# CTPLab/Tera-MIND

Hardware: AMD Instinct MI355X
Metric: denoising steps/sec on 64x64x(2 stains x 2 z) patches (interior patch-steps/s) (higher is better)
Workload: dtype f32; 1 GPU; configs[1]: b=32 images x 1 interior 64x64 patch (P=1, 128 padded + 32 collage patches/step), rna_slc=4, rna_num=229, stain=all, DDPM T=50 schedule, f32, mode A (pad+patchify -> UNet -> DDPM update); parallelism=dp1 (independent patch batches)

## Files before the change

### include/teramind_hip.h

```cpp
#ifndef TERAMIND_HIP_H
#define TERAMIND_HIP_H

#include <stddef.h>
#include <stdint.h>

#ifdef __cplusplus
extern "C" {
#endif

#define TM_ABI_VERSION 1

enum {
  TM_OK = 0,
  TM_ERR_ARG = -1,
  TM_ERR_STATE = -2,
  TM_ERR_KEY = -3,
  TM_ERR_HIP = -4,
  TM_ERR_WORKSPACE = -5
};

enum { TM_DTYPE_F32 = 0, TM_DTYPE_BF16 = 1, TM_DTYPE_F16 = 2 };
enum { TM_SAMPLE_DDPM = 0, TM_SAMPLE_DDIM = 1 };

typedef struct tm_config {
// ... 138 lines not shown
  double total_ms;
  double nominal_flops;
  double executed_flops;
  double alg_bytes;
} tm_prof_stats;
int tm_profile_enable(tm_model* m, int on);
int tm_profile_collect(tm_model* m, tm_prof_stats* out);


int tm_op_to_cb8(const void* x_ncdhw, void* y_cb8, int N, int C, int Z, int H, int W, void* stream);
int tm_op_from_cb8(const void* x_cb8, void* y_ncdhw, int N, int C, int Z, int H, int W, void* stream);

int tm_op_conv_mfma(const void* x_cb8, const void* w_host, const void* bias_host, void* y_cb8,
                    int N, int Cin, int Cout, int Z, int S, int ksize, int zmode, int up2,
                    int tile_variant, void* stream);
int tm_op_conv_mfma_res(const void* x_cb8, const void* w_host, const void* bias_host, void* y_cb8, const void* res_cb8,
                        int res_half, int N, int Cin, int Cout, int Z, int S, int ksize, int zmode, int up2,
                        int tile_variant, void* stream);

int tm_op_conv_zpair_fused_f32(const void* x_cb8, const void* w_host, const void* bias_host, const void* norm_w_host,
                               const void* scale_host, const void* shift_host, const void* res_cb8, void* a2_out,
                               void* h1_out, void* a2_sep_out, int N, int Cin, int Cout, int Z, int S, int per_image,
                               int tile_variant, void* stream);

int tm_op_conv_ups_pair_f32(const void* x_cb8, const void* w_host, const void* bias_host, void* y_cb8, int N, int Cin,
                            int Cout, int Z, int S, int tile_variant, void* stream);

int tm_op_conv_xpair_f32(const void* x_cb8, const void* w_host, const void* bias_host, void* y_cb8, const void* res_cb8,
                         int res_half, int N, int Cin, int Cout, int Z, int S, int tile_variant, void* stream);
int tm_op_conv_pad1_time_f32(const void* x_cb8, const void* w_host, const void* bias_host, void* y_cb8, int N, int Cin,
                             int Cout, int S, int form, int tile_variant, int iters, float* ms_out, void* stream);

int tm_op_conv1_f32(const void* x_cb8, const void* w_host, const void* bias_host, void* y_cb8, const void* res_cb8,
                    const void* gate_cb8, int x_cbtot, int x_cb0, int gate_cbtot, int gate_cb0, int gate_half, int gelu,
                    int tile_variant, int N, int Cin, int Cout, int Z, int S, int* form_out, void* stream);
int tm_conv1_form(long vox, int ntile, int tile_variant);

int tm_conv_frag_addrs(int kernel, int half, int tw, int what, int wave, int p, int ky, int kx, int sub, int* out64);

int tm_op_conv27_bf16(const void* x_cb8, const void* w_host, const void* bias_host, void* y_cb8,
                      int N, int Cin, int Cout, int S, int dtype, int waves, const void* res_h16, void* y_h16,
                      int ups, int res_half, void* stream);
int tm_op_conv27_h16_z(const void* x_cb8, const void* w_host, const void* bias_host, void* y_cb8,
                       int N, int Cin, int Cout, int S, int dtype, int waves, const void* res_h16, void* y_h16,
                       int ups, int res_half, int Z, void* stream);

// ... 135 lines not shown
```

### tera-mind_amd/_lib.py

```python
import ctypes as C
import os

_HERE = os.path.dirname(os.path.abspath(__file__))
LIB_PATH = os.environ.get("TM_LIB_PATH") or os.path.join(_HERE, "csrc", "libteramind_hip.so")

c_void_p, c_int, c_size_t, c_char_p, c_float = C.c_void_p, C.c_int, C.c_size_t, C.c_char_p, C.c_float
c_i64_p = C.POINTER(C.c_int64)


class TmConfig(C.Structure):
    _fields_ = [("patch_size", C.c_int32), ("rna_slc", C.c_int32), ("n_stain", C.c_int32),
                ("rna_num", C.c_int32), ("net_ch", C.c_int32), ("ch_mult", C.c_int32 * 4),
                ("embed_ch", C.c_int32), ("attn_res", C.c_int32), ("num_res_blocks", C.c_int32),
                ("vis_only", C.c_int32), ("dtype", C.c_int32)]


class TmStepCoefs(C.Structure):
    _fields_ = [("sqrt_recip_alphas_cumprod", c_float), ("sqrt_recipm1_alphas_cumprod", c_float),
                ("posterior_mean_coef1", c_float), ("posterior_mean_coef2", c_float),
                ("sigma", c_float), ("sqrt_alpha_bar_prev", c_float),
                ("sqrt_one_minus_alpha_bar_prev", c_float)]


class TmProfStats(C.Structure):
# ... 50 lines not shown
                                        C.c_int64, c_void_p, c_void_p]),
    "tm_blosc_frame_info": (c_int, [c_void_p, c_size_t, c_void_p]),
    "tm_blosc_decompress_dev": (c_int, [c_void_p, c_void_p, c_void_p, c_int, c_void_p, C.c_int64, c_void_p, c_void_p, c_void_p]),
    "tm_blosc_decompress_tiles": (c_int, [c_void_p, c_void_p, c_void_p, c_int, c_void_p, c_int] + [C.c_int64] * 3 + [c_void_p] * 3),
    "tm_u8_shrink2": (c_int, [c_void_p, c_int, c_int, C.c_int64, c_void_p, C.c_int64, c_void_p]),
    "tm_jpeg_encode_tiles": (c_int, [c_void_p, c_int, c_int, C.c_int64] + [c_int] * 3 + [c_void_p, C.c_int64] + [c_void_p] * 4),
    "tm_jpeg_tables": (c_int, [c_int, c_void_p, c_size_t, C.POINTER(c_size_t)]),
    "tm_ssim_planes": (c_int, [c_void_p, c_void_p] + [c_int] * 4 + [C.c_int64] * 4 + [C.POINTER(c_float), c_int, c_float, c_float, c_void_p, c_void_p]),
    "tm_avgpool2_pad": (c_int, [c_void_p] + [c_int] * 4 + [C.c_int64] * 2 + [c_void_p] + [C.c_int64] * 2 + [c_void_p]),
    "tm_profile_enable": (c_int, [c_void_p, c_int]),
    "tm_profile_collect": (c_int, [c_void_p, C.POINTER(TmProfStats)]),
    "tm_op_to_cb8": (c_int, [c_void_p, c_void_p, c_int, c_int, c_int, c_int, c_int, c_void_p]),
    "tm_op_from_cb8": (c_int, [c_void_p, c_void_p, c_int, c_int, c_int, c_int, c_int, c_void_p]),
    "tm_op_conv_mfma": (c_int, [c_void_p, c_void_p, c_void_p, c_void_p] + [c_int] * 9 + [c_void_p]),
    "tm_op_conv_mfma_res": (c_int, [c_void_p, c_void_p, c_void_p, c_void_p, c_void_p] + [c_int] * 10 + [c_void_p]),
    "tm_op_conv1_f32": (c_int, [c_void_p] * 6 + [c_int] * 12 + [C.POINTER(c_int), c_void_p]),
    "tm_conv1_form": (c_int, [C.c_long, c_int, c_int]),
    "tm_conv_frag_addrs": (c_int, [c_int] * 9 + [c_void_p]),
    "tm_op_conv27_bf16": (c_int, [c_void_p, c_void_p, c_void_p, c_void_p] + [c_int] * 6 + [c_void_p] * 2 + [c_int] * 2 + [c_void_p]),
    "tm_op_conv27_fused": (c_int, [c_void_p] * 7 + [c_int] * 7 + [c_void_p]),
    "tm_op_conv27_h16_z": (c_int, [c_void_p, c_void_p, c_void_p, c_void_p] + [c_int] * 6 + [c_void_p] * 2 + [c_int] * 3 + [c_void_p]),
    "tm_op_conv27_fused_z": (c_int, [c_void_p] * 7 + [c_int] * 8 + [c_void_p]),
    "tm_op_conv_zpair_fused_f32": (c_int, [c_void_p] * 10 + [c_int] * 7 + [c_void_p]),
    "tm_op_conv_ups_pair_f32": (c_int, [c_void_p] * 4 + [c_int] * 6 + [c_void_p]),
    "tm_op_conv_xpair_f32": (c_int, [c_void_p] * 5 + [c_int] * 7 + [c_void_p]),
    "tm_op_conv_pad1_time_f32": (c_int, [c_void_p] * 4 + [c_int] * 7 + [C.POINTER(c_float), c_void_p]),
    "tm_op_conv27_time":(c_int, [c_int] * 10 + [c_void_p, c_void_p]),
    "tm_op_conv1_bf16": (c_int, [c_void_p, c_void_p, c_void_p, c_void_p] + [c_int] * 8 + [c_void_p] * 4),
    "tm_op_conv1_h16_gate": (c_int, [c_void_p, c_void_p, c_void_p, c_void_p] + [c_int] * 8 + [c_void_p] * 3 + [c_int] * 3 + [c_void_p]),
    "tm_op_conv1_concat": (c_int, [c_void_p, c_void_p, c_void_p, c_int, c_void_p, c_void_p, c_void_p] + [c_int] * 8 + [c_void_p]),
    "tm_op_prep_h16": (c_int, [c_void_p] * 3 + [c_int] * 7 + [c_void_p, c_int, c_int, c_void_p, c_void_p, C.c_long] +
                       [c_int] * 4 + [c_void_p, c_void_p, c_int, c_void_p, c_void_p]),
    "tm_op_prep_f32": (c_int, [c_void_p] * 3 + [c_int] * 7 + [c_void_p, c_int, c_int, c_void_p, c_void_p, C.c_long] +
                       [c_int] * 4 + [c_void_p, c_void_p, c_int, c_void_p, c_void_p]),
    "tm_op_prep_form": (c_int, [c_void_p] * 3 + [c_int] * 9 + [c_void_p, c_int, c_int, c_int, c_void_p, c_void_p, C.c_long] +
                        [c_int] * 5 + [c_void_p, c_void_p, c_int, c_int, c_void_p, c_void_p]),
    "tm_op_stem": (c_int, [c_void_p] * 4 + [c_int] * 6 + [c_void_p]),
    "tm_op_head": (c_int, [c_void_p] * 4 + [c_int] * 6 + [c_void_p]),
    "tm_op_time_embed": (c_int, [c_void_p] * 7 + [c_int] * 3 + [c_void_p]),
    "tm_op_emb_all": (c_int, [c_void_p] * 4 + [c_int] * 3 + [c_void_p]),
    "tm_op_prep_train": (c_int, [c_void_p] * 5 + [c_float, c_int, c_void_p] + [c_int] * 4 + [c_void_p]),
    "tm_op_prep_bwd": (c_int, [c_void_p] * 6 + [c_float, c_int] + [c_void_p] * 4 + [c_int] * 4 + [c_void_p]),
    "tm_op_prep_train_rng": (c_int, [c_void_p] * 4 + [C.c_uint64, C.c_uint, c_float, c_int, c_void_p] + [c_int] * 4 + [c_void_p]),
    "tm_op_prep_bwd_rng": (c_int, [c_void_p] * 5 + [C.c_uint64, C.c_uint, c_float, c_int] + [c_void_p] * 4 + [c_int] * 4 + [c_void_p]),
    "tm_op_dropout_mask": (c_int, [C.c_uint64, C.c_uint, c_float, c_void_p] + [c_int] * 4 + [c_void_p]),
    "tm_op_conv_dgrad": (c_int, [c_void_p, c_void_p, c_void_p] + [c_int] * 6 + [c_void_p]),
# ... 63 lines not shown
```

### tera-mind_amd/csrc/tm_conv_pack.cpp

```cpp
#include "tm_conv_frag.h"
#include "tm_kernels.h"

#include <stdlib.h>
#include <string.h>

#include <vector>

namespace tmk {

int conv_form_taps(int form) {
  switch (form) {
    case CF_1X1: return 1;
    case CF_INPLANE: return 9;
    case CF_ZSKIP_UPS: case CF_PAIR_UPS: return 12;
    case CF_XPAIR: return 36;
    default: return 27;
  }
}
static bool form_ups(int form) { return form == CF_ZSKIP_UPS || form == CF_PAIR_UPS; }
size_t conv_pack_floats(int form, int Cout, int Cbi) {
  return (size_t)(form_ups(form) ? 4 : 1) * ((Cout + 63) / 64) * Cbi * conv_form_taps(form) * 512;
}
ConvW conv_w(int form, int Cout, int Cbi) {
  ConvW cw;
  cw.form = form; cw.Cout = Cout; cw.Cbi = Cbi; cw.taps = conv_form_taps(form); cw.ntile = (Cout + 63) / 64;
  return cw;
}

static bool switch_on(const char* name) {
  const char* v = getenv(name);
  return !(v && atoi(v) == 0);
}
int conv_pick_form(int ksize, int zmode, int Z, bool deep8, int role, bool* fuse_mid) {
  static const bool zpair_on = switch_on("TM_CONV_ZPAIR"), xpair_on = switch_on("TM_CONV_XPAIR"),
                    xmid_on = switch_on("TM_CONV_XPAIR_MID"), fuse_on = switch_on("TM_CONV_FUSE_MID");
  if (fuse_mid) *fuse_mid = false;
  if (ksize == 1) return CF_1X1;
  if (zmode == ZM_INPLANE) return CF_INPLANE;
  if (zmode == ZM_VALID) return CF_PLANES3;
  const bool pair = Z == 2 && zpair_on;
  if (zmode == ZM_UPS) return ((role & ROLE_OP_PAIR_UPS) || ((role & ROLE_RES) && pair)) ? CF_PAIR_UPS : CF_ZSKIP_UPS;
  if (Z != 2) return (Z == 1 && (role & ROLE_RES)) ? CF_INPLANE : CF_PLANES3;
  if ((role & ROLE_OP_XPAIR) && xpair_on) return CF_XPAIR;
  if (!pair) return CF_ZSKIP;
  const bool fuses = (role & ROLE_C1_64) && fuse_on;
  const bool xp = (role & ROLE_RES) && !(role & ROLE_DEEP) && xpair_on && deep8 && (!fuses || xmid_on);
  if (fuse_mid) *fuse_mid = fuses && !xp;
  return xp ? CF_XPAIR : CF_PAIR;
}

static void seg_counts(const int* seg_c, int nseg, int& Cin, int& Cbi) {
  Cin = Cbi = 0;
  for (int s = 0; s < nseg; ++s) { Cin += seg_c[s]; Cbi += (seg_c[s] + 7) / 8; }
}
static void pack_taps(const float* w, int Cout, const int* seg_c, int nseg, int taps, float* out, bool halves = false) {
  int Cin, Cbi;
  seg_counts(seg_c, nseg, Cin, Cbi);
  memset(out, 0, (size_t)((Cout + 63) / 64) * Cbi * taps * 512 * sizeof(float));
  int ci0 = 0, cb0 = 0;
  for (int s = 0; s < nseg; ++s) {
    for (int c = 0; c < seg_c[s]; ++c) {
      const int ci = ci0 + c;
      const int cb = cb0 + c / 8, c8 = c % 8;
      for (int co = 0; co < Cout; ++co) {
        const int nt = co / 64, col = co % 64;
        const float* src = w + ((size_t)co * Cin + ci) * taps;
        float* dst = out + (((size_t)nt * Cbi + cb) * taps) * 512 + (halves ? conv_w_off(col, c8) : col * 8 + c8);
        for (int t = 0; t < taps; ++t) dst[(size_t)t * 512] = src[t];
      }
    }
// ... 88 lines not shown
```

### tera-mind_amd/csrc/tm_device.h

```cpp
#pragma once
#include "tm_kernels.h"
#include <math.h>
#include <atomic>

namespace tmk {

typedef float f32x4 __attribute__((ext_vector_type(4)));
typedef float f32x16 __attribute__((ext_vector_type(16)));

#define TM_EPS 1e-6f

struct DevOnce {
  std::atomic<unsigned long long> done[2] = {{0ull}, {0ull}};
  static int dev() { int d = -1; return hipGetDevice(&d) == hipSuccess ? d : -1; }
  bool need() const {
    const int d = dev();
    if (d < 0 || d >= 128) return true;
    return !((done[d >> 6].load(std::memory_order_acquire) >> (d & 63)) & 1ull);
  }
  void mark() {
    const int d = dev();
    if (d >= 0 && d < 128) done[d >> 6].fetch_or(1ull << (d & 63), std::memory_order_release);
  }
};
// ... 184 lines not shown
  const float t = h ? t1 : t0;
  if (ooff < 0) return;
  const float rstd = 1.0f / sqrtf(t * a.inv_c + TM_EPS);
  const long mo = (long)(n / a.per_image) * a.mod_stride;
  float* yp = a.y + (long)n * a.y_nstride + ooff + 4 * h;
#pragma unroll
  for (int ct = 0; ct < 2; ++ct)
#pragma unroll
    for (int g = 0; g < 4; ++g) {
      const int c0 = (ct * 4 + g) * 8 + 4 * h;
      const f32x4 wn = *(const f32x4*)(a.norm_w + c0);
      const f32x4 sc = *(const f32x4*)(a.mod_scale + mo + c0), sh = *(const f32x4*)(a.mod_shift + mo + c0);
      f32x4 r;
#pragma unroll
      for (int j = 0; j < 4; ++j) {
        float v = wn[j] * (o[ct][0][4 * g + j] * rstd);
        v = v * (1.0f + sc[j]) + sh[j];
        r[j] = silu_h16(v);
      }
      *(f32x4*)(yp + (long)(ct * 4 + g) * a.y_plane) = r;
    }
}

}
```

### tera-mind_amd/csrc/tm_kernels.h

```cpp
#pragma once
#include <hip/hip_runtime.h>
#include <stdint.h>

#include <vector>

#include "../../include/teramind_hip.h"

namespace tmk {

struct TV {
  float* p = nullptr;
  int N = 0, C = 0, Cb = 0, Z = 0, H = 0, W = 0;
  long nstride = 0;
  long plane() const { return (long)Z * H * W * 8; }
  TV blocks(int cb0, int ncb) const {
    TV v = *this;
    v.p = p + (long)cb0 * plane();
    v.Cb = ncb;
    v.C = ncb * 8;
    return v;
  }
};
inline TV cb8_view(void* p, int N, int C, int Z, int H, int W) {
  TV t;
// ... 37 lines not shown
enum { EPI_NONE = 0, EPI_GELU = 1, EPI_UP2 = 2 };
enum { ZM_PAD1 = 0, ZM_INPLANE = 1, ZM_VALID = 2,
       ZM_UPS = 3 };
struct ConvLaunch {
  TV x;
  ConvW w;
  TV y;
  const TV* res = nullptr;
  const TV* gate = nullptr;
  int flags = 0;
  int tile_variant = 0;
  int gate_half = 0;
  int res_half = 0;
  int zmode = ZM_PAD1;
  int fuse_norm = 0;
  const float *norm_w = nullptr, *mod_scale = nullptr, *mod_shift = nullptr;
  float inv_c = 0.f;
  long mod_stride = 0;
  int per_image = 1;
  TV a2;
};
hipError_t launch_conv_mfma(const ConvLaunch& L, hipStream_t s);
int conv_tile(int form, long ovox, int ntile, int S, int tile_variant);
int conv_frag_addrs(int kernel, int half, int tw, int what, int wv, int p, int ky, int kx, int sub, int* out);
int conv1_form(long vox, int ntile, int tile_variant);

struct TVH {
  uint16_t* p = nullptr;
  int N = 0, C = 0, Cb = 0, Z = 0, H = 0, W = 0;
  long nstride = 0;
  TVH blocks(int cb0, int ncb) const {
    TVH t = *this;
    t.p = p + (long)cb0 * Z * H * W * 8;
    t.Cb = ncb; t.C = ncb * 8;
    return t;
  }
};
struct ConvLaunchH {
  TVH x;
  const uint16_t* w = nullptr;
  const float* bias = nullptr;
  int Cout = 0;
  TV y;
  const TV* res = nullptr;
  const TV* gate = nullptr;
  const TVH* gate_h = nullptr;
// ... 291 lines not shown
```

### tera-mind_amd/csrc/tm_kernels.hip

```cpp
#include "tm_conv_pair.h"

#include <stdlib.h>
#include <string.h>

#include <type_traits>

namespace tmk {

template <int NZI, int WM, int TW, bool UPS = false>
struct C3Geo {
  static constexpr int TW_ = TW;
  static constexpr int MV = 4 * WM * 32;
  static constexpr int TR = (MV / TW < TW) ? (MV / TW) : TW;
  static constexpr int NPB = MV / (TR * TW);
  static constexpr int HR = TR + 2, HC = TW + 2;
  static constexpr int XV = NPB * NZI * HR * HC;
  static constexpr int XPIECES = XV * 2;
  static constexpr int PX = (XPIECES + 255) / 256;
  static constexpr int TZ = UPS ? 4 : 9;
  static constexpr int NTAP = TZ * NZI;
  static constexpr int WFLOATS = NTAP * 512;
  static constexpr int WPIECES = WFLOATS / 4;
  static constexpr int PW = (WPIECES + 255) / 256;
  static constexpr int TAPS_TOTAL = (NZI == 1) ? 9 : 3 * TZ;
// ... 433 lines not shown
  conv_epilogue<1, NC>(a, o, nte, h, on, ooff1, 0);
}

template <int HALF, int TW>
struct XPGeo {
  static constexpr int TW_ = TW;
  static constexpr int NW = 4;
  static constexpr int NQ = HALF ? 2 : 4;
  static constexpr int MP = HALF ? 32 : 64;
  static constexpr int PWD = TW / 2;
  static constexpr int TR = (MP / PWD < TW) ? (MP / PWD) : TW;
  static constexpr int NPB = MP / (TR * PWD);
  static constexpr int HR = TR + 2;
  static constexpr int XP = NPB * HR * PWD;
  static constexpr int XITEMS = XP * 2;
  static_assert(XP % 8 == 0, "whole groups of eight staging items (tm_conv_frag.h)");
  static constexpr int WSLOT = 12 * 512;
  static constexpr int KP = 24 / NW;
  static constexpr int LDS_BYTES = (2 * WSLOT + 12 * XP * 8) * 4;
};
template <class G>
TM_HD constexpr int xp_xtap(int p, int q, int ky) { return (p * 4 + q) * G::XP * 8 + conv_frag_off(ky * G::PWD, 0, G::XP); }

template <int HALF, int TW>
__global__ __launch_bounds__(256, 2) void conv3d_xpair(ConvArgs a) {
  using G = XPGeo<HALF, TW>;
  static_assert(G::XITEMS <= 64 * G::NW, "one staging item per thread");
  extern __shared__ __attribute__((aligned(16))) float lds[];
  float* lw = lds;

  const int tid = threadIdx.x;
  const int lane = tid & 63, wv = tid >> 6;
  const int i32 = lane & 31, h = lane >> 5;

  const int S = a.S;
  const ConvTile t = conv_tile_of<TW, G::TR, false, false>(a);
  const int nt = t.nt, pg = t.pg, tr = t.tr, tc = t.tc;

  long xoff = -1;
  bool okl = false, okr = false;
  if (tid < G::XITEMS) {
    const int half = conv_stage_half(tid);
    int v = conv_stage_row(tid);
    const int j = v % G::PWD; v /= G::PWD;
    const int hr = v % G::HR;
    const int ps = v / G::HR;
    const int n = pg * G::NPB + ps;
    const int y = tr * G::TR + hr - 1, x = tc * TW + 2 * j;
// ... 135 lines not shown
      }
#pragma unroll
    for (int p = 0; p < 3; ++p) {
      acc[p][0] = qh ? (got[p] - acc[p][0]) - acc[p][1] : (acc[p][0] + acc[p][1]) + got[p];
      asm volatile("" : "+v"(acc[p][0]));
    }
#pragma unroll
    for (int z = 0; z < 2; ++z) {
      f32x16 o[1][1];
      o[0][0] = acc[0][0] + acc[1 + z][0];
      asm volatile("" : "+v"(o[0][0]));
      const int ooff[1] = {ooff0 >= 0 ? ooff0 + (z * S * S + qh) * 8 : -1};
      __builtin_amdgcn_sched_barrier(0);
      conv_epilogue<1, 1>(a, o, nte, h, on, ooff, 2 * S);
    }
  } else {
#pragma unroll
    for (int p = 0; p < 3; ++p) {
      const f32x16 ev = (acc[p][0] + acc[p][1]) + acc[p][2];
      acc[p][1] = (acc[p][1] - acc[p][2]) - acc[p][3];
      acc[p][0] = ev;
      asm volatile("" : "+v"(acc[p][0]), "+v"(acc[p][1]));
    }
#pragma unroll
    for (int z = 0; z < 2; ++z)
#pragma unroll
      for (int par = 0; par < 2; ++par) {
        f32x16 o[1][1];
        o[0][0] = acc[0][par] + acc[1 + z][par];
        asm volatile("" : "+v"(o[0][0]));
        const int ooff[1] = {ooff0 >= 0 ? ooff0 + (z * S * S + par) * 8 : -1};
        __builtin_amdgcn_sched_barrier(0);
        conv_epilogue<1, 1>(a, o, nte, h, on, ooff, 2 * S);
      }
  }
}

template <int WM, int WN>
__global__ __launch_bounds__(256, 2) void conv1_mfma(ConvArgs a) {
  constexpr int MV = 4 * WM * 32;
  constexpr int KC = 4;
  constexpr int XP = KC * MV * 2 / 256;
  constexpr int NT64 = WN / 2;
  constexpr int WP = NT64 * KC * 64 * 2 / 256;
  __shared__ __attribute__((aligned(16))) float lds[NT64 * KC * 512 + KC * MV * 8];
  float* lw = lds;
  float* lx = lds + NT64 * KC * 512;

  const int tid = threadIdx.x;
  const int lane = tid & 63, wv = tid >> 6;
  const int i32 = lane & 31, h = lane >> 5;
  const int bid = xcd_swizzle(blockIdx.x, gridDim.x);
  const int nt = bid % a.ntile;
  const int mtile = bid / a.ntile;
  const long VPN = (long)a.Z * a.S * a.S;
  const long vtot = VPN * a.N;

// ... 76 lines not shown
        for (int ct = 0; ct < WN; ++ct)
#pragma unroll
          for (int mt = 0; mt < WM; ++mt)
            acc[ct][mt] = __builtin_amdgcn_mfma_f32_32x32x2f32(wf[ct][kk], xf[mt][kk], acc[ct][mt], 0, 0, 0);
    }
  }
  conv_epilogue<WM, WN>(a, acc, nt, h, on, ooff, 0);
}

static bool conv_fills_chip(long vox, long tiles) { return (vox / 256) * tiles >= 512; }

int conv1_form(long vox, int ntile, int tile_variant) {
  if (tile_variant == 3) return (ntile & 1) == 0 ? 3 : 0;
  const int variant = tile_variant ? tile_variant : (conv_fills_chip(vox, ntile) ? 2 : 1);
  if (variant == 2 && (ntile & 1) == 0 && conv_fills_chip(vox, ntile / 2)) return 3;
  return variant == 2 ? 2 : 1;
}

int conv_tile(int form, long ovox, int ntile, int S, int tile_variant) {
  if (S == 4) return 1;
  const long tiles = (form == CF_ZSKIP_UPS || form == CF_PAIR_UPS) ? 4L * ntile : ntile;
  const int variant = tile_variant ? tile_variant : (conv_fills_chip(ovox, tiles) ? 2 : 1);
  return variant == 2 ? 2 : 1;
}

template <void (*KERN)(ConvArgs), class G, int BLOCK = 256>
static hipError_t launch_tiled(const ConvArgs& a, long factor, hipStream_t s) {
  static DevOnce attr_once;
  if (attr_once.need()) {
    hipError_t e = hipFuncSetAttribute((const void*)KERN, hipFuncAttributeMaxDynamicSharedMemorySize, G::LDS_BYTES);
    if (e != hipSuccess) return e;
    attr_once.mark();
  }
  const long tiles = (long)(a.S / G::TW_) * (a.S / G::TR);
  const long pgs = (a.N + G::NPB - 1) / G::NPB;
  hipLaunchKernelGGL(KERN, dim3((unsigned)(pgs * tiles * factor * a.ntile)), dim3(BLOCK), G::LDS_BYTES, s, a);
  return hipGetLastError();
}
template <int MAXTW, class F>
static hipError_t with_tile_width(int S, F f) {
  if constexpr (MAXTW >= 32)
    if (S >= 32) return f(std::integral_constant<int, 32>{});
  if (S >= 16) return f(std::integral_constant<int, 16>{});
  return f(std::integral_constant<int, 8>{});
}
template <int NZI, bool UPS>
// ... 5 lines not shown
    return large ? launch_tiled<conv3d_mfma<NZI, 2, TW, UPS>, C3Geo<NZI, 2, TW, UPS>>(a, factor, s)
                 : launch_tiled<conv3d_mfma<NZI, 1, TW, UPS>, C3Geo<NZI, 1, TW, UPS>>(a, factor, s);
  });
}

hipError_t launch_conv_mfma(const ConvLaunch& L, hipStream_t s) {
  ConvArgs a;
  a.x = L.x.p; a.x_nstride = L.x.nstride; a.x_plane = L.x.plane();
  a.w = L.w.w; a.bias = L.w.bias;
  a.y = L.y.p; a.y_nstride = L.y.nstride; a.y_plane = L.y.plane(); a.Cob = L.y.Cb;
  a.res = L.res ? L.res->p : nullptr; a.res_nstride = L.res ? L.res->nstride : 0;
  a.gate = L.gate ? L.gate->p : nullptr; a.gate_nstride = L.gate ? L.gate->nstride : 0;
  const int form = L.w.form;
  if (L.w.taps != conv_form_taps(form)) return hipErrorInvalidValue;
  if (L.gate_half) {
    int ls = 0;
    while ((1 << ls) < L.y.H) ++ls;
    if (!L.gate || form != CF_1X1 || (1 << ls) != L.y.H || L.y.H != L.y.W || ls < 1) return hipErrorInvalidValue;
    a.gate_ls = ls;
  }
  a.N = L.x.N; a.S = L.x.H; a.Z = L.x.Z; a.Cbi = L.w.Cbi; a.ntile = L.w.ntile; a.flags = L.flags;
  if (L.x.Cb != L.w.Cbi || L.x.H != L.x.W) return hipErrorInvalidValue;
  if (L.fuse_norm) {
    if (form != CF_PAIR || L.zmode != ZM_PAD1 || L.x.Z != 2 || L.w.Cout != 64 || L.w.ntile != 1 || L.res || L.gate || L.flags ||
        !L.norm_w || !L.mod_scale || !L.mod_shift || L.per_image < 1)
      return hipErrorInvalidValue;
    if (conv_tile(form, (long)L.x.N * 2 * L.x.H * L.x.H, 1, L.x.H, L.tile_variant) != 2) return hipErrorInvalidValue;
    if (!L.a2.p || L.a2.Cb != 8 || L.a2.N != L.x.N || L.a2.Z != 2 || L.a2.H != L.x.H || L.a2.W != L.x.H) return hipErrorInvalidValue;
    if (L.y.Cb != 8 || L.y.Z != 2 || L.y.H != L.x.H) return hipErrorInvalidValue;
    a.y = L.a2.p; a.y_nstride = L.a2.nstride; a.y_plane = L.a2.plane();
    a.norm_w = L.norm_w; a.mod_scale = L.mod_scale; a.mod_shift = L.mod_shift; a.mod_stride = L.mod_stride;
    a.per_image = L.per_image; a.inv_c = L.inv_c;
  }
  if (L.y.Cb > L.w.ntile * 8 || L.y.N != L.x.N) return hipErrorInvalidValue;
  const long vox = (long)a.N * a.Z * a.S * a.S;
  if (form == CF_1X1) {
    if (L.flags & EPI_UP2) return hipErrorInvalidValue;
    if (L.y.H != L.x.H || L.y.Z != L.x.Z) return hipErrorInvalidValue;
    const int form1 = conv1_form(vox, a.ntile, L.tile_variant);
    if (form1 == 3) {
      const long mt = (vox + 255) / 256;
      a.ntile /= 2;
      hipLaunchKernelGGL((conv1_mfma<2, 4>), dim3((unsigned)(mt * a.ntile)), dim3(256), 0, s, a);
    } else if (form1 == 2) {
      const long mt = (vox + 255) / 256;
      hipLaunchKernelGGL((conv1_mfma<2, 2>), dim3((unsigned)(mt * a.ntile)), dim3(256), 0, s, a);
    } else if (form1 == 1) {
      const long mt = (vox + 127) / 128;
      hipLaunchKernelGGL((conv1_mfma<1, 2>), dim3((unsigned)(mt * a.ntile)), dim3(256), 0, s, a);
    } else return hipErrorInvalidValue;
// ... 34 lines not shown
  switch (form) {
    case CF_INPLANE: return launch_c3<1, false>(a, large, s);
    case CF_PLANES3: return launch_c3<3, false>(a, large, s);
    case CF_ZSKIP: return launch_c3<2, false>(a, large, s);
    case CF_ZSKIP_UPS: return launch_c3<2, true>(a, large, s);
    case CF_PAIR:
      if (S == 4) return launch_tiled<conv3d_zpair<1, 4, false>, ZPGeo<1, 4>>(a, 1, s);
      return with_tile_width<32>(S, [&](auto tw) {
        constexpr int TW = decltype(tw)::value;
        if (L.fuse_norm) return launch_tiled<conv3d_zpair<0, TW, true>, ZPGeo<0, TW>>(a, 1, s);
        return large ? launch_tiled<conv3d_zpair<0, TW, false>, ZPGeo<0, TW>>(a, 1, s)
                     : launch_tiled<conv3d_zpair<1, TW, false>, ZPGeo<1, TW>>(a, 1, s);
      });
    case CF_PAIR_UPS:
      if (S == 4) return launch_tiled<conv3d_zpair_ups<1, 4>, ZPUGeo<1, 4>>(a, 4, s);
      return with_tile_width<32>(S, [&](auto tw) {
        constexpr int TW = decltype(tw)::value;
        return large ? launch_tiled<conv3d_zpair_ups<0, TW>, ZPUGeo<0, TW>>(a, 4, s)
                     : launch_tiled<conv3d_zpair_ups<1, TW>, ZPUGeo<1, TW>>(a, 4, s);
      });
    default:
      return with_tile_width<16>(S, [&](auto tw) {
        constexpr int TW = decltype(tw)::value;
        return large ? launch_tiled<conv3d_xpair<0, TW>, XPGeo<0, TW>, 64 * XPGeo<0, TW>::NW>(a, 1, s)
                     : launch_tiled<conv3d_xpair<1, TW>, XPGeo<1, TW>, 64 * XPGeo<1, TW>::NW>(a, 1, s);
      });
  }
}

template <class G, int HALF, int TW, bool UPS>
static int zpair_frag_addrs(int what, int wv, int p, int ky, int kx, int sub, int* out) {
  constexpr int NC = HALF ? 1 : 2, KW = UPS ? 2 : 3;
  constexpr int lx = G::LDS_BYTES / 4 - 3 * G::XV * 8;
  if (p < 0 || p > 2) return -1;
  if (what == 2 ? (ky < 0 || ky >= G::PX) : (ky < 0 || ky >= KW || kx < 0 || kx >= KW)) return -1;
  if (what == 0 ? (sub < 0 || sub >= NC) : what == 1 ? (sub < 0 || sub > (UPS ? 3 : 0)) : false) return -1;
  const int vt = HALF ? (wv & 1) : wv, ct0 = HALF ? (wv >> 1) : 0;
  for (int lane = 0; lane < 64; ++lane) {
    const int i32 = lane & 31, h = lane >> 5;
    int a = -1;
    if (what == 0) a = zp_wtap(UPS ? p * 4 + ky * 2 + kx : p * 9 + ky * 3 + kx, sub) + conv_w_off(ct0 * 32 + i32, 4 * h);
    else if (what == 1)
      a = lx + zp_xtap<G>(p, ky, kx) + conv_lane_of<G::TR, TW, G::PS, G::HC, G::XV>(vt * 32 + conv_lane_voxel(TW, i32), h, sub >> 1, sub & 1).xb;
    else {
      const int i = wv * 64 + lane + ky * 256;
      if (conv_stage_row(i) < G::XV) a = lx + p * G::XV * 8 + conv_frag_off(conv_stage_row(i), conv_stage_half(i), G::XV);
// ... 1009 lines not shown
```

### tera-mind_amd/csrc/tm_model.hip

```cpp
#include "../../include/teramind_hip.h"
#include "tm_kernels.h"

#include <algorithm>
#include <cmath>
#include <map>
#include <string>
#include <type_traits>
#include <vector>
#include <stdarg.h>
#include <stdio.h>
#include <stdlib.h>
#include <string.h>

using namespace tmk;

static thread_local char g_err[512] = "";
int tmk::fail(int code, const char* fmt, ...) {
  va_list ap;
  va_start(ap, fmt);
  vsnprintf(g_err, sizeof(g_err), fmt, ap);
  va_end(ap);
  return code;
}

// ... 862 lines not shown
    TV A2 = cx.tensor(N, w.cout, Z, S_out), H1 = cx.tensor(N, w.cout, Z, S_out);
    ConvLaunch L1 = conv(A, w.c1u, H1);
    L1.zmode = ZM_UPS;
    run_conv(cx, L1);
    PrepLaunch Q = mid_section(cx, w, H1, per_image);
    prep_out(Q, A2);
    cx.run(Q);
    ConvLaunch L2 = conv(A2, w.c2, out);
    L2.res = &src[0].t; L2.res_half = 1;
    run_conv(cx, L2, w.cout);
    cx.top = mark;
    return out;
  }
  int cin_pad = w.cbi * 8;
  TV A = cx.tensor(N, cin_pad, Z, S_out), raw;
  const bool need_raw = w.has_skip || mode != RS_SAME || src.size() > 1 || src[0].collage;
  if (need_raw) raw = cx.tensor(N, cin_pad, Z, S_out);
  PrepLaunch P = block_input(cx, w, src, N, Z, S_out, per_image, mode);
  prep_out(P, A);
  if (need_raw) prep_raw(P, raw);
  cx.run(P);
  TV A2 = cx.tensor(N, w.cout, Z, S_out);
  ConvLaunch L1 = conv(A, w.c1, A2);
  if (w.fuse_mid && Z == 2 && conv_tile(CF_PAIR, (long)N * Z * S_out * S_out, 1, S_out, 0) == 2) {
    fuse_mid_section(L1, cx, w, per_image, A2);
    run_conv(cx, L1, w.cin);
  } else {
    TV H1 = cx.tensor(N, w.cout, Z, S_out);
    L1.y = H1;
    run_conv(cx, L1, w.cin);
    PrepLaunch Q = mid_section(cx, w, H1, per_image);
    prep_out(Q, A2);
    cx.run(Q);
  }
  if (w.has_skip) run_conv(cx, conv(raw, w.skip, out));
  ConvLaunch L2 = conv(A2, w.c2, out);
  L2.res = w.has_skip ? &out : (need_raw ? &raw : &src[0].t);
  run_conv(cx, L2, w.cout);
  cx.top = mark;
  return out;
}

struct AttnGeom { bool half = false, mfma_core = false; int Sc = 0; };
struct AttnCond {
  TV mod, kv;
  TVH mod_h, kv_h;
};
// ... 587 lines not shown
```

### tera-mind_amd/csrc/tm_ops.hip

```cpp
#include "../../include/teramind_hip.h"
#include "tm_kernels.h"

#include <algorithm>
#include <cmath>
#include <cstdint>
#include <tuple>
#include <utility>
#include <vector>
#include <string.h>

using namespace tmk;

struct DevTmp {
  std::vector<void*> ptrs;
  std::vector<hipEvent_t> events;
  hipError_t err = hipSuccess;
  const char* what = "";
  bool ordered = false;
  hipStream_t st = nullptr;
  DevTmp() = default;
  explicit DevTmp(hipStream_t stream) : ordered(true), st(stream) { keep_pool(); }
  static void keep_pool() {
    static bool done[64] = {};
    int dev = 0;
// ... 132 lines not shown
    L.res_half = res_half ? 1 : 0;
  }
  return TM_OK;
}

extern "C" int tm_op_conv_mfma_res(const void* x_cb8, const void* w_host, const void* bias_host, void* y_cb8, const void* res_cb8,
                                   int res_half, int N, int Cin, int Cout, int Z, int S, int ksize, int zmode, int up2,
                                   int tile_variant, void* stream) {
  if (ksize != 1 && ksize != 3) return fail(TM_ERR_ARG, "ksize must be 1 or 3");
  if (zmode != ZM_PAD1 && zmode != ZM_INPLANE && zmode != ZM_VALID && zmode != ZM_UPS) return fail(TM_ERR_ARG, "bad zmode");
  const bool ups = ksize == 3 && zmode == ZM_UPS;
  if (zmode == ZM_UPS && (ksize != 3 || up2)) return fail(TM_ERR_ARG, "ZM_UPS: ksize 3, no fused upsample of the output");
  if (res_cb8 && (ksize != 3 || zmode == ZM_UPS)) return fail(TM_ERR_ARG, "residual: k x 3 x 3 forms other than ZM_UPS only");
  if (res_half && (!res_cb8 || up2 || S < 2)) return fail(TM_ERR_ARG, "res_half: needs a residual, S >= 2 and no fused upsample");
  const int Zout = (ksize == 3 && zmode == ZM_VALID) ? Z - 2 : Z;
  ConvOp op;
  if (const int rc = conv_op(op, conv_pick_form(ksize, zmode, Z, false, ROLE_OP), w_host, bias_host, x_cb8, y_cb8, N, Cin, Cout, Z, S,
                             Zout, (up2 || ups) ? 2 * S : S, zmode, tile_variant, res_cb8, res_half))
    return rc;
  op.L.flags = up2 ? EPI_UP2 : 0;
  return finish((hipStream_t)stream, launch_conv_mfma(op.L, (hipStream_t)stream), "conv_mfma");
}

extern "C" int tm_op_conv_zpair_fused_f32(const void* x_cb8, const void* w_host, const void* bias_host, const void* norm_w_host,
                                          const void* scale_host, const void* shift_host, const void* res_cb8, void* a2_out,
                                          void* h1_out, void* a2_sep_out, int N, int Cin, int Cout, int Z, int S, int per_image,
                                          int tile_variant, void* stream) {
  if (!x_cb8 || !w_host || !bias_host || !norm_w_host || !scale_host || !shift_host || !a2_out) return fail(TM_ERR_ARG, "null argument");
  if (N < 1 || Cin < 1 || per_image < 1) return fail(TM_ERR_ARG, "N, Cin, per_image must be positive");
  if (Z != 2) return fail(TM_ERR_ARG, "the pair form exists at Z == 2 only (got Z = %d)", Z);
  if (Cout != 64) return fail(TM_ERR_ARG, "the fused mid-section needs Cout == 64: one wave holds every channel (got %d)", Cout);
  if (res_cb8) return fail(TM_ERR_ARG, "the fused mid-section takes no residual");
  if (S != 8 && S != 16 && S != 32 && S != 64 && S != 128) return fail(TM_ERR_ARG, "S must be 8, 16, 32, 64 or 128 (got %d)", S);
  if (tile_variant < 0 || tile_variant > 2) return fail(TM_ERR_ARG, "tile_variant must be 0 (auto), 1 or 2 (got %d)", tile_variant);
  if (conv_tile(CF_PAIR, (long)N * Z * S * S, 1, S, tile_variant) != 2)
    return fail(TM_ERR_ARG, "the fused mid-section exists in the 128-voxel tile only; this launch takes the 64-voxel one");
  if (a2_sep_out && !h1_out) return fail(TM_ERR_ARG, "a2_sep_out needs h1_out");
  if (conv_pick_form(3, ZM_PAD1, Z, false, ROLE_OP) != CF_PAIR) return fail(TM_ERR_ARG, "the pair form is switched off (TM_CONV_ZPAIR=0)");
  ConvOp op;
  if (const int rc = conv_op(op, CF_PAIR, w_host, bias_host, x_cb8, a2_out, N, Cin, Cout, Z, S, Z, S, ZM_PAD1, tile_variant)) return rc;
  const int nimg = (N + per_image - 1) / per_image;
  const float* nw = op.tmp.alloc((size_t)Cout, (const float*)norm_w_host);
  const float* sc = op.tmp.alloc((size_t)nimg * Cout, (const float*)scale_host);
  const float* sh = op.tmp.alloc((size_t)nimg * Cout, (const float*)shift_host);
  if (op.tmp.err) return op.tmp.report();
  hipStream_t st = (hipStream_t)stream;
  ConvLaunch& L = op.L;
  L.fuse_norm = 1; L.a2 = L.y; L.norm_w = nw; L.mod_scale = sc; L.mod_shift = sh; L.mod_stride = Cout; L.per_image = per_image;
  L.inv_c = 1.0f / (float)Cout;
  hipError_t e = launch_conv_mfma(L, st);
  if (e == hipSuccess && h1_out) {
    ConvLaunch U = L;
    U.fuse_norm = 0; U.y = cb8_view(h1_out, N, Cout, Z, S, S);
    e = launch_conv_mfma(U, st);
    if (e == hipSuccess && a2_sep_out) {
      PrepLaunch P = prep_start(N, Z, S);
      prep_src(P, U.y);
      prep_norm(P, nw, Cout);
      P.mod = MOD_IMAGE; P.mod_scale = sc; P.mod_shift = sh; P.mod_stride = Cout;
      P.act = 1; P.per_image = per_image;
      prep_out(P, cb8_view(a2_sep_out, N, Cout, Z, S, S));
      e = launch_prep(P, st);
    }
  }
  return finish(st, e, "conv_zpair_fused (fp32)");
}

extern "C" int tm_op_conv_ups_pair_f32(const void* x_cb8, const void* w_host, const void* bias_host, void* y_cb8, int N, int Cin,
                                       int Cout, int Z, int S, int tile_variant, void* stream) {
  if (!x_cb8 || !w_host || !bias_host || !y_cb8) return fail(TM_ERR_ARG, "null argument");
  if (N < 1 || Cin < 1 || Cout < 1) return fail(TM_ERR_ARG, "N, Cin, Cout must be positive");
  if (Z != 2) return fail(TM_ERR_ARG, "the pair form exists at Z == 2 only (got Z = %d)", Z);
  if (S != 4 && S != 8 && S != 16 && S != 32 && S != 64) return fail(TM_ERR_ARG, "S must be 4, 8, 16, 32 or 64 (got %d)", S);
  if (tile_variant < 0 || tile_variant > 2) return fail(TM_ERR_ARG, "tile_variant must be 0 (auto), 1 or 2 (got %d)", tile_variant);
  ConvOp op;
  if (const int rc = conv_op(op, conv_pick_form(3, ZM_UPS, Z, false, ROLE_OP_PAIR_UPS), w_host, bias_host, x_cb8, y_cb8, N, Cin, Cout, Z,
                             S, Z, 2 * S, ZM_UPS, tile_variant))
    return rc;
  return finish((hipStream_t)stream, launch_conv_mfma(op.L, (hipStream_t)stream), "conv_ups_pair (fp32)");
}

static int xpair_args(const void* x, const void* w, const void* b, const void* y, int N, int Cin, int Cout, int Z, int S,
                      int tile_variant) {
  if (!x || !w || !b || !y) return fail(TM_ERR_ARG, "null argument");
  if (N < 1 || Cin < 1 || Cout < 1) return fail(TM_ERR_ARG, "N, Cin, Cout must be positive");
  if (Z != 2) return fail(TM_ERR_ARG, "the x-pair form exists at Z == 2 only (got Z = %d)", Z);
  if (S != 8 && S != 16 && S != 32 && S != 64 && S != 128) return fail(TM_ERR_ARG, "S must be 8, 16, 32, 64 or 128 (got %d)", S);
  if (tile_variant < 0 || tile_variant > 2) return fail(TM_ERR_ARG, "tile_variant must be 0 (auto), 1 or 2 (got %d)", tile_variant);
// ... 1303 lines not shown
```

Before: 945.7 interior patch-steps/s.

## Fuse norm, modulation and SiLU epilogue into the x-pair conv kernel

Adds a fused epilogue to the x-pair 3x3x3 conv kernel that computes the channel RMS norm across the two waves holding each half of the channels, exchanging partial sums through LDS. It then applies the norm weight, per-image scale/shift and SiLU before writing. With the new TM_CONV_XPAIR_FUSE switch on by default, res blocks that pick the x-pair form keep the mid-section fusion instead of dropping it. This removes a separate prep/norm pass and a round trip of the conv output through memory, at the cost of extra syncthreads and LDS traffic inside the conv. A new TM_CONV_XPAIR_DEEP switch, off by default, gates x-pair use in deep layers.

New measurement: 955.1 interior patch-steps/s (median of 6 runs). Within noise of the previous version (+1.0%).

```diff
diff --git a/include/teramind_hip.h b/include/teramind_hip.h
--- a/include/teramind_hip.h
+++ b/include/teramind_hip.h
@@ -184,6 +184,10 @@
                                const void* scale_host, const void* shift_host, const void* res_cb8, void* a2_out,
                                void* h1_out, void* a2_sep_out, int N, int Cin, int Cout, int Z, int S, int per_image,
                                int tile_variant, void* stream);
+int tm_op_conv_xpair_fused_f32(const void* x_cb8, const void* w_host, const void* bias_host, const void* norm_w_host,
+                               const void* scale_host, const void* shift_host, const void* res_cb8, void* a2_out,
+                               void* h1_out, void* a2_sep_out, int N, int Cin, int Cout, int Z, int S, int per_image,
+                               int tile_variant, void* stream);
 
 int tm_op_conv_ups_pair_f32(const void* x_cb8, const void* w_host, const void* bias_host, void* y_cb8, int N, int Cin,
                             int Cout, int Z, int S, int tile_variant, void* stream);
diff --git a/tera-mind_amd/_lib.py b/tera-mind_amd/_lib.py
--- a/tera-mind_amd/_lib.py
+++ b/tera-mind_amd/_lib.py
@@ -96,6 +96,7 @@
     "tm_op_conv27_h16_z": (c_int, [c_void_p, c_void_p, c_void_p, c_void_p] + [c_int] * 6 + [c_void_p] * 2 + [c_int] * 3 + [c_void_p]),
     "tm_op_conv27_fused_z": (c_int, [c_void_p] * 7 + [c_int] * 8 + [c_void_p]),
     "tm_op_conv_zpair_fused_f32": (c_int, [c_void_p] * 10 + [c_int] * 7 + [c_void_p]),
+    "tm_op_conv_xpair_fused_f32": (c_int, [c_void_p] * 10 + [c_int] * 7 + [c_void_p]),
     "tm_op_conv_ups_pair_f32": (c_int, [c_void_p] * 4 + [c_int] * 6 + [c_void_p]),
     "tm_op_conv_xpair_f32": (c_int, [c_void_p] * 5 + [c_int] * 7 + [c_void_p]),
     "tm_op_conv_pad1_time_f32": (c_int, [c_void_p] * 4 + [c_int] * 7 + [C.POINTER(c_float), c_void_p]),
diff --git a/tera-mind_amd/csrc/tm_conv_pack.cpp b/tera-mind_amd/csrc/tm_conv_pack.cpp
--- a/tera-mind_amd/csrc/tm_conv_pack.cpp
+++ b/tera-mind_amd/csrc/tm_conv_pack.cpp
@@ -27,13 +27,14 @@
   return cw;
 }
 
-static bool switch_on(const char* name) {
+static bool switch_on(const char* name, bool dflt = true) {
   const char* v = getenv(name);
-  return !(v && atoi(v) == 0);
+  return v ? atoi(v) != 0 : dflt;
 }
 int conv_pick_form(int ksize, int zmode, int Z, bool deep8, int role, bool* fuse_mid) {
   static const bool zpair_on = switch_on("TM_CONV_ZPAIR"), xpair_on = switch_on("TM_CONV_XPAIR"),
-                    xmid_on = switch_on("TM_CONV_XPAIR_MID"), fuse_on = switch_on("TM_CONV_FUSE_MID");
+                    xmid_on = switch_on("TM_CONV_XPAIR_MID"), fuse_on = switch_on("TM_CONV_FUSE_MID"),
+                    xfuse_on = switch_on("TM_CONV_XPAIR_FUSE"), xdeep_on = switch_on("TM_CONV_XPAIR_DEEP", false);
   if (fuse_mid) *fuse_mid = false;
   if (ksize == 1) return CF_1X1;
   if (zmode == ZM_INPLANE) return CF_INPLANE;
@@ -44,8 +45,9 @@
   if ((role & ROLE_OP_XPAIR) && xpair_on) return CF_XPAIR;
   if (!pair) return CF_ZSKIP;
   const bool fuses = (role & ROLE_C1_64) && fuse_on;
-  const bool xp = (role & ROLE_RES) && !(role & ROLE_DEEP) && xpair_on && deep8 && (!fuses || xmid_on);
-  if (fuse_mid) *fuse_mid = fuses && !xp;
+  const bool deep_pair = (role & ROLE_DEEP) && !xdeep_on;
+  const bool xp = (role & ROLE_RES) && !deep_pair && xpair_on && deep8 && (!fuses || xmid_on);
+  if (fuse_mid) *fuse_mid = fuses && (!xp || xfuse_on);
   return xp ? CF_XPAIR : CF_PAIR;
 }
 
diff --git a/tera-mind_amd/csrc/tm_device.h b/tera-mind_amd/csrc/tm_device.h
--- a/tera-mind_amd/csrc/tm_device.h
+++ b/tera-mind_amd/csrc/tm_device.h
@@ -230,4 +230,62 @@
     }
 }
 
-}
+__device__ __forceinline__ void xpair_norm_epilogue(const ConvArgs& a, const f32x16 (&acc)[3][4], float* lds, int wv, int lane,
+                                                    int n, int ooff0, int S2) {
+  const int h = lane >> 5, ch = wv & 1;
+  f32x4 bv[4];
+#pragma unroll
+  for (int g = 0; g < 4; ++g) bv[g] = *(const f32x4*)(a.bias + (ch * 4 + g) * 8 + 4 * h);
+  f32x4 s8[4];
+  __syncthreads();
+#pragma unroll
+  for (int t = 0; t < 4; ++t) {
+    const f32x16 o = acc[0][t & 1] + acc[1 + (t >> 1)][t & 1];
+#pragma unroll
+    for (int g = 0; g < 4; ++g) {
+      float p[4];
+#pragma unroll
+      for (int j = 0; j < 4; ++j) {
+        const float v = o[4 * g + j] + bv[g][j];
+        p[j] = v * v;
+        asm volatile("" : "+v"(p[j]));
+      }
+      const float lo = ((p[0] + p[1]) + p[2]) + p[3];
+      const float lo_p = __shfl_xor(lo, 32, 64);
+      s8[t][g] = (((lo_p + p[0]) + p[1]) + p[2]) + p[3];
+    }
+    *(f32x4*)(lds + ((wv * 4 + t) * 64 + lane) * 4) = s8[t];
+  }
+  __syncthreads();
+  const long mo = (long)(n / a.per_image) * a.mod_stride;
+#pragma unroll
+  for (int t = 0; t < 4; ++t) {
+    const f32x4 got = *(const f32x4*)(lds + (((wv ^ 1) * 4 + t) * 64 + lane) * 4);
+    float red[4];
+#pragma unroll
+    for (int r = 0; r < 4; ++r) red[r] = s8[t][r] + got[r];
+    const float t1 = ((red[0] + red[1]) + red[2]) + red[3];
+    const float t0 = __shfl_xor(t1, 32, 64);
+    const float ts = h ? t1 : t0;
+    if (ooff0 < 0) continue;
+    const float rstd = 1.0f / sqrtf(ts * a.inv_c + TM_EPS);
+    const f32x16 o = acc[0][t & 1] + acc[1 + (t >> 1)][t & 1];
+    float* yp = a.y + (long)n * a.y_nstride + ooff0 + (t >> 1) * S2 + (t & 1) * 8 + 4 * h;
+#pragma unroll
+    for (int g = 0; g < 4; ++g) {
+      const int c0 = (ch * 4 + g) * 8 + 4 * h;
+      const f32x4 wn = *(const f32x4*)(a.norm_w + c0);
+      const f32x4 sc = *(const f32x4*)(a.mod_scale + mo + c0), sh = *(const f32x4*)(a.mod_shift + mo + c0);
+      f32x4 r;
+#pragma unroll
+      for (int j = 0; j < 4; ++j) {
+        float v = wn[j] * ((o[4 * g + j] + bv[g][j]) * rstd);
+        v = v * (1.0f + sc[j]) + sh[j];
+        r[j] = silu_h16(v);
+      }
+      *(f32x4*)(yp + (long)(ch * 4 + g) * a.y_plane) = r;
+    }
+  }
+}
+
+}
diff --git a/tera-mind_amd/csrc/tm_kernels.h b/tera-mind_amd/csrc/tm_kernels.h
--- a/tera-mind_amd/csrc/tm_kernels.h
+++ b/tera-mind_amd/csrc/tm_kernels.h
@@ -83,6 +83,7 @@
 };
 hipError_t launch_conv_mfma(const ConvLaunch& L, hipStream_t s);
 int conv_tile(int form, long ovox, int ntile, int S, int tile_variant);
+bool conv_fuse_tile(int form, long ovox, int S, int tile_variant);
 int conv_frag_addrs(int kernel, int half, int tw, int what, int wv, int p, int ky, int kx, int sub, int* out);
 int conv1_form(long vox, int ntile, int tile_variant);
 
diff --git a/tera-mind_amd/csrc/tm_kernels.hip b/tera-mind_amd/csrc/tm_kernels.hip
--- a/tera-mind_amd/csrc/tm_kernels.hip
+++ b/tera-mind_amd/csrc/tm_kernels.hip
@@ -479,8 +479,9 @@
 template <class G>
 TM_HD constexpr int xp_xtap(int p, int q, int ky) { return (p * 4 + q) * G::XP * 8 + conv_frag_off(ky * G::PWD, 0, G::XP); }
 
-template <int HALF, int TW>
+template <int HALF, int TW, bool FUSE = false>
 __global__ __launch_bounds__(256, 2) void conv3d_xpair(ConvArgs a) {
+  static_assert(!FUSE || HALF == 0, "the fused mid-section needs both cout halves of a voxel in one workgroup");
   using G = XPGeo<HALF, TW>;
   static_assert(G::XITEMS <= 64 * G::NW, "one staging item per thread");
   extern __shared__ __attribute__((aligned(16))) float lds[];
@@ -662,17 +663,21 @@
       acc[p][0] = ev;
       asm volatile("" : "+v"(acc[p][0]), "+v"(acc[p][1]));
     }
-#pragma unroll
-    for (int z = 0; z < 2; ++z)
-#pragma unroll
-      for (int par = 0; par < 2; ++par) {
-        f32x16 o[1][1];
-        o[0][0] = acc[0][par] + acc[1 + z][par];
-        asm volatile("" : "+v"(o[0][0]));
-        const int ooff[1] = {ooff0 >= 0 ? ooff0 + (z * S * S + par) * 8 : -1};
-        __builtin_amdgcn_sched_barrier(0);
-        conv_epilogue<1, 1>(a, o, nte, h, on, ooff, 2 * S);
-      }
+    if constexpr (FUSE) {
+      xpair_norm_epilogue(a, acc, lds, wv, lane, on[0], ooff0, S * S * 8);
+    } else {
+#pragma unroll
+      for (int z = 0; z < 2; ++z)
+#pragma unroll
+        for (int par = 0; par < 2; ++par) {
+          f32x16 o[1][1];
+          o[0][0] = acc[0][par] + acc[1 + z][par];
+          asm volatile("" : "+v"(o[0][0]));
+          const int ooff[1] = {ooff0 >= 0 ? ooff0 + (z * S * S + par) * 8 : -1};
+          __builtin_amdgcn_sched_barrier(0);
+          conv_epilogue<1, 1>(a, o, nte, h, on, ooff, 2 * S);
+        }
+    }
   }
 }
 
@@ -795,6 +800,11 @@
   const long tiles = (form == CF_ZSKIP_UPS || form == CF_PAIR_UPS) ? 4L * ntile : ntile;
   const int variant = tile_variant ? tile_variant : (conv_fills_chip(ovox, tiles) ? 2 : 1);
   return variant == 2 ? 2 : 1;
+}
+
+bool conv_fuse_tile(int form, long ovox, int S, int tile_variant) {
+  if (form != CF_PAIR && !(form == CF_XPAIR && S >= 16)) return false;
+  return conv_tile(form, ovox, 1, S, tile_variant) == 2;
 }
 
 template <void (*KERN)(ConvArgs), class G, int BLOCK = 256>
@@ -846,10 +856,10 @@
   a.N = L.x.N; a.S = L.x.H; a.Z = L.x.Z; a.Cbi = L.w.Cbi; a.ntile = L.w.ntile; a.flags = L.flags;
   if (L.x.Cb != L.w.Cbi || L.x.H != L.x.W) return hipErrorInvalidValue;
   if (L.fuse_norm) {
-    if (form != CF_PAIR || L.zmode != ZM_PAD1 || L.x.Z != 2 || L.w.Cout != 64 || L.w.ntile != 1 || L.res || L.gate || L.flags ||
+    if ((form != CF_PAIR && form != CF_XPAIR) || L.zmode != ZM_PAD1 || L.x.Z != 2 || L.w.Cout != 64 || L.w.ntile != 1 || L.res || L.gate || L.flags ||
         !L.norm_w || !L.mod_scale || !L.mod_shift || L.per_image < 1)
       return hipErrorInvalidValue;
-    if (conv_tile(form, (long)L.x.N * 2 * L.x.H * L.x.H, 1, L.x.H, L.tile_variant) != 2) return hipErrorInvalidValue;
+    if (!conv_fuse_tile(form, (long)L.x.N * 2 * L.x.H * L.x.H, L.x.H, L.tile_variant)) return hipErrorInvalidValue;
     if (!L.a2.p || L.a2.Cb != 8 || L.a2.N != L.x.N || L.a2.Z != 2 || L.a2.H != L.x.H || L.a2.W != L.x.H) return hipErrorInvalidValue;
     if (L.y.Cb != 8 || L.y.Z != 2 || L.y.H != L.x.H) return hipErrorInvalidValue;
     a.y = L.a2.p; a.y_nstride = L.a2.nstride; a.y_plane = L.a2.plane();
@@ -930,6 +940,8 @@
     default:
       return with_tile_width<16>(S, [&](auto tw) {
         constexpr int TW = decltype(tw)::value;
+        if constexpr (TW == 16)
+          if (L.fuse_norm) return launch_tiled<conv3d_xpair<0, 16, true>, XPGeo<0, 16>, 64 * XPGeo<0, 16>::NW>(a, 1, s);
         return large ? launch_tiled<conv3d_xpair<0, TW>, XPGeo<0, TW>, 64 * XPGeo<0, TW>::NW>(a, 1, s)
                      : launch_tiled<conv3d_xpair<1, TW>, XPGeo<1, TW>, 64 * XPGeo<1, TW>::NW>(a, 1, s);
       });
diff --git a/tera-mind_amd/csrc/tm_model.hip b/tera-mind_amd/csrc/tm_model.hip
--- a/tera-mind_amd/csrc/tm_model.hip
+++ b/tera-mind_amd/csrc/tm_model.hip
@@ -908,7 +908,7 @@
   cx.run(P);
   TV A2 = cx.tensor(N, w.cout, Z, S_out);
   ConvLaunch L1 = conv(A, w.c1, A2);
-  if (w.fuse_mid && Z == 2 && conv_tile(CF_PAIR, (long)N * Z * S_out * S_out, 1, S_out, 0) == 2) {
+  if (w.fuse_mid && Z == 2 && conv_fuse_tile(w.c1.form, (long)N * Z * S_out * S_out, S_out, 0)) {
     fuse_mid_section(L1, cx, w, per_image, A2);
     run_conv(cx, L1, w.cin);
   } else {
diff --git a/tera-mind_amd/csrc/tm_ops.hip b/tera-mind_amd/csrc/tm_ops.hip
--- a/tera-mind_amd/csrc/tm_ops.hip
+++ b/tera-mind_amd/csrc/tm_ops.hip
@@ -178,23 +178,26 @@
   return finish((hipStream_t)stream, launch_conv_mfma(op.L, (hipStream_t)stream), "conv_mfma");
 }
 
-extern "C" int tm_op_conv_zpair_fused_f32(const void* x_cb8, const void* w_host, const void* bias_host, const void* norm_w_host,
-                                          const void* scale_host, const void* shift_host, const void* res_cb8, void* a2_out,
-                                          void* h1_out, void* a2_sep_out, int N, int Cin, int Cout, int Z, int S, int per_image,
-                                          int tile_variant, void* stream) {
+static int conv_fused_op(int form, const void* x_cb8, const void* w_host, const void* bias_host, const void* norm_w_host,
+                         const void* scale_host, const void* shift_host, const void* res_cb8, void* a2_out, void* h1_out,
+                         void* a2_sep_out, int N, int Cin, int Cout, int Z, int S, int per_image, int tile_variant, void* stream) {
+  const bool xp = form == CF_XPAIR;
+  const char* name = xp ? "x-pair" : "pair";
   if (!x_cb8 || !w_host || !bias_host || !norm_w_host || !scale_host || !shift_host || !a2_out) return fail(TM_ERR_ARG, "null argument");
   if (N < 1 || Cin < 1 || per_image < 1) return fail(TM_ERR_ARG, "N, Cin, per_image must be positive");
-  if (Z != 2) return fail(TM_ERR_ARG, "the pair form exists at Z == 2 only (got Z = %d)", Z);
-  if (Cout != 64) return fail(TM_ERR_ARG, "the fused mid-section needs Cout == 64: one wave holds every channel (got %d)", Cout);
+  if (Z != 2) return fail(TM_ERR_ARG, "the %s form exists at Z == 2 only (got Z = %d)", name, Z);
+  if (Cout != 64) return fail(TM_ERR_ARG, "the fused mid-section needs Cout == 64: one workgroup holds every channel (got %d)", Cout);
   if (res_cb8) return fail(TM_ERR_ARG, "the fused mid-section takes no residual");
-  if (S != 8 && S != 16 && S != 32 && S != 64 && S != 128) return fail(TM_ERR_ARG, "S must be 8, 16, 32, 64 or 128 (got %d)", S);
+  if ((xp || S != 8) && S != 16 && S != 32 && S != 64 && S != 128)
+    return fail(TM_ERR_ARG, "S must be %s16, 32, 64 or 128 (got %d)", xp ? "" : "8, ", S);
   if (tile_variant < 0 || tile_variant > 2) return fail(TM_ERR_ARG, "tile_variant must be 0 (auto), 1 or 2 (got %d)", tile_variant);
-  if (conv_tile(CF_PAIR, (long)N * Z * S * S, 1, S, tile_variant) != 2)
+  if (!conv_fuse_tile(form, (long)N * Z * S * S, S, tile_variant))
     return fail(TM_ERR_ARG, "the fused mid-section exists in the 128-voxel tile only; this launch takes the 64-voxel one");
   if (a2_sep_out && !h1_out) return fail(TM_ERR_ARG, "a2_sep_out needs h1_out");
-  if (conv_pick_form(3, ZM_PAD1, Z, false, ROLE_OP) != CF_PAIR) return fail(TM_ERR_ARG, "the pair form is switched off (TM_CONV_ZPAIR=0)");
+  if (xp ? conv_pick_form(3, ZM_PAD1, 2, true, ROLE_OP_XPAIR) != CF_XPAIR : conv_pick_form(3, ZM_PAD1, Z, false, ROLE_OP) != CF_PAIR)
+    return fail(TM_ERR_ARG, "the %s form is switched off (%s=0)", name, xp ? "TM_CONV_XPAIR" : "TM_CONV_ZPAIR");
   ConvOp op;
-  if (const int rc = conv_op(op, CF_PAIR, w_host, bias_host, x_cb8, a2_out, N, Cin, Cout, Z, S, Z, S, ZM_PAD1, tile_variant)) return rc;
+  if (const int rc = conv_op(op, form, w_host, bias_host, x_cb8, a2_out, N, Cin, Cout, Z, S, Z, S, ZM_PAD1, tile_variant)) return rc;
   const int nimg = (N + per_image - 1) / per_image;
   const float* nw = op.tmp.alloc((size_t)Cout, (const float*)norm_w_host);
   const float* sc = op.tmp.alloc((size_t)nimg * Cout, (const float*)scale_host);
@@ -219,7 +222,21 @@
       e = launch_prep(P, st);
     }
   }
-  return finish(st, e, "conv_zpair_fused (fp32)");
+  return finish(st, e, xp ? "conv_xpair_fused (fp32)" : "conv_zpair_fused (fp32)");
+}
+extern "C" int tm_op_conv_zpair_fused_f32(const void* x_cb8, const void* w_host, const void* bias_host, const void* norm_w_host,
+                                          const void* scale_host, const void* shift_host, const void* res_cb8, void* a2_out,
+                                          void* h1_out, void* a2_sep_out, int N, int Cin, int Cout, int Z, int S, int per_image,
+                                          int tile_variant, void* stream) {
+  return conv_fused_op(CF_PAIR, x_cb8, w_host, bias_host, norm_w_host, scale_host, shift_host, res_cb8, a2_out, h1_out, a2_sep_out, N,
+                       Cin, Cout, Z, S, per_image, tile_variant, stream);
+}
+extern "C" int tm_op_conv_xpair_fused_f32(const void* x_cb8, const void* w_host, const void* bias_host, const void* norm_w_host,
+                                          const void* scale_host, const void* shift_host, const void* res_cb8, void* a2_out,
+                                          void* h1_out, void* a2_sep_out, int N, int Cin, int Cout, int Z, int S, int per_image,
+                                          int tile_variant, void* stream) {
+  return conv_fused_op(CF_XPAIR, x_cb8, w_host, bias_host, norm_w_host, scale_host, shift_host, res_cb8, a2_out, h1_out, a2_sep_out, N,
+                       Cin, Cout, Z, S, per_image, tile_variant, stream);
 }
 
 extern "C" int tm_op_conv_ups_pair_f32(const void* x_cb8, const void* w_host, const void* bias_host, void* y_cb8, int N, int Cin,
```
